# lyclyc52/NeRF_RPN

Hardware: AMD Instinct MI355X
Metric: scenes/sec (160^3x4 grids, VGG19-3D+FPN+RPN fwd+bwd) (higher is better)
Workload: dtype bf16; 1 GPU; configs[1]: one 160x160x160x4 rgb-sigma grid per GPU, VGG19-EF 3D + FPN + anchor RPN (OBB, 16 GT boxes per scene), fwd+bwd+clip+AdamW, random-init weights; scenes_per_gpu=1, parallelism=dp1, world_size_seen=1, backend=single process

## Files before the change

### include/nerfrpn.h

```cpp
#ifndef NERFRPN_H
#define NERFRPN_H

#include <stddef.h>
#include <stdint.h>

#ifdef __cplusplus
extern "C" {
#endif

typedef void *nrpn_stream_t;

enum nrpn_status {
  NRPN_OK = 0,
  NRPN_ERR_ARG = -1,
  NRPN_ERR_LAUNCH = -2,
  NRPN_ERR_DEVICE = -3
};

enum nrpn_dtype { NRPN_F32 = 0, NRPN_BF16 = 1 };

const char *nrpn_last_error(void);
int nrpn_abi_version(void);
int nrpn_check_device(int ordinal);

// ... 233 lines not shown
int nrpn_roipool_obb_bwd(const float *dout, const int32_t *argmax, const float *rois, const int32_t *level_of, int level, int num_rois,
                         float scale, int interpolation, int x, int y, int z, int c, int o0, int o1, int o2, void *dfeat, void *workspace,
                         int dtype, nrpn_stream_t stream);

int nrpn_a2a_reduce_bf16(const void *recv, const float *local, int rank, int world, int64_t chunk, void *out, nrpn_stream_t stream);
int nrpn_grad_sumsq_floats(void);
int nrpn_grad_sumsq(const float *grad, int64_t count, float grad_scale, float *sumsq, nrpn_stream_t stream);
int nrpn_adamw_step(float *param, const float *grad, float *exp_avg, float *exp_avg_sq, int64_t count,
                    const float *sumsq, float grad_scale, float max_norm, float lr, float beta1, float beta2, float eps,
                    float weight_decay, int step, void *shadow_bf16, nrpn_stream_t stream);
int nrpn_adamw_step_zero_grad(float *param, float *grad, float *exp_avg, float *exp_avg_sq, int64_t count,
                              const float *sumsq, float grad_scale, float max_norm, float lr, float beta1, float beta2, float eps,
                              float weight_decay, int step, void *shadow_bf16, nrpn_stream_t stream);
int nrpn_transpose_weights(const float *master, void *dst, const int64_t *table, const int32_t *tile_prefix, int nweights,
                           int total_tiles, int dtype, nrpn_stream_t stream);
int nrpn_reduce_slices(const float *partials, int slices, int64_t count, float *dst, int accumulate, const float *bias_partials,
                       int wrows, int cout, float *gbias, int accumulate_bias, nrpn_stream_t stream);
size_t nrpn_conv3d_wgrad_bias_offset(int n, int gx, int gy, int gz, int ksize);

enum nrpn_heatmap_kernel { NRPN_HEATMAP_GAUSSIAN = 0, NRPN_HEATMAP_BOX = 1 };
int nrpn_heatmap_splat(const int32_t *aabbs, int num_boxes, const double *factors, const int32_t *factor_offsets, int kernel_type,
                       int x, int y, int z, float *out, nrpn_stream_t stream);
int nrpn_gaussian_filter3d(const float *in, int x, int y, int z, float sigma, int radius, const double *weights, float *work, float *out,
                           nrpn_stream_t stream);
int nrpn_heatmap_work_doubles(void);
int nrpn_heatmap_standardize(const float *in, int64_t n, double *work, float *out, float *mean_std, nrpn_stream_t stream);
int nrpn_render_mip(const float *heatmap, int x, int y, int z, int downsample, float value_scale, const double *cams, int num_frames,
                    const double *jet, int width, int height, double *work, uint8_t *rgb, float *mip, nrpn_stream_t stream);

int nrpn_zoom_cubic3d(const float *in, int nx, int ny, int nz, const double *h_zpow, int ox, int oy, int oz, double *coef, float *out,
// ... 68 lines not shown
```

### include/nerfrpn_tools.h

```cpp
#ifndef NERFRPN_TOOLS_H
#define NERFRPN_TOOLS_H
#include "nerfrpn.h"

#ifdef __cplusplus
extern "C" {
#endif

int nrpn_set_conv_kstep_bytes(int kb);
int nrpn_set_conv_lds_dma(int on);
int nrpn_set_conv_tile_m(int bm);
int nrpn_set_conv_halo_auto(int on);
int nrpn_set_conv_halo_pairing(int mode);
int nrpn_set_conv_stagger(int on);
int nrpn_set_conv_big_split(int on);
int nrpn_set_wgrad_big_tile(int on);
int nrpn_set_wgrad_pack2(int on);
int nrpn_set_sumsq_form(int form, int grid);
int nrpn_set_wgrad_transpose_read(int on);
int nrpn_set_rows_big_tile(int on);
int nrpn_set_rows_tail_split(int on);
int nrpn_set_bn_fast(int on);
int nrpn_set_bn_reduce_v8(int on);
int nrpn_set_pool_fast(int on);
int nrpn_set_gn_fast(int on);
int64_t nrpn_fastdiv_host(int64_t n, int64_t d);
int nrpn_set_window_attn_mfma(int on);

#ifdef __cplusplus
}
#endif
#endif
```

### nerf_rpn_amd/csrc/common.h

```cpp
#pragma once
#include <hip/hip_runtime.h>
#include <hip/hip_bf16.h>

#include <cstdarg>
#include <cstdint>
#include <cstdio>

#include "../../include/nerfrpn.h"
#include "../../include/nerfrpn_tools.h"

int nrpn_fail(int code, const char *fmt, ...);

#define NRPN_REQUIRE(cond, ...)                                 \
  do {                                                          \
    if (!(cond)) return nrpn_fail(NRPN_ERR_ARG, __VA_ARGS__);   \
  } while (0)

#define NRPN_HIP(call)                                                                          \
  do {                                                                                          \
    hipError_t e_ = (call);                                                                     \
    if (e_ != hipSuccess) return nrpn_fail(NRPN_ERR_LAUNCH, "%s: %s", #call, hipGetErrorString(e_)); \
  } while (0)

#define NRPN_LAUNCH_CHECK(name)                                                                  \
// ... 11 lines not shown
  unsigned l = 0;
  while ((1ull << l) < d) ++l;
  f.m = (unsigned)((((unsigned long long)1 << (31 + l)) + d - 1) / d);
  f.sh = l - 1;
  return f;
}
__device__ __forceinline__ unsigned fastdiv(unsigned n, const FastDiv &f) { return f.d == 1 ? n : (__umulhi(n, f.m) >> f.sh); }


int nrpn_ensure_dynamic_lds(const void *kernel, int bytes);
#define NRPN_LDS(kernel, bytes)                                                                         \
  do {                                                                                                  \
    if (int rc_ = nrpn_ensure_dynamic_lds(reinterpret_cast<const void *>(kernel), (int)(bytes))) return rc_; \
  } while (0)

static inline hipStream_t as_stream(nrpn_stream_t s) { return reinterpret_cast<hipStream_t>(s); }
static inline int64_t cdiv64(int64_t a, int64_t b) { return (a + b - 1) / b; }

__device__ __forceinline__ float bf16_bits_to_f32(unsigned short h) { return __uint_as_float(((unsigned)h) << 16); }
__device__ __forceinline__ unsigned short f32_to_bf16_bits(float f) { return __builtin_bit_cast(unsigned short, (__bf16)f); }

template <typename T> struct elem;
template <> struct elem<float> {
  static __device__ __forceinline__ float ld(const float *p) { return *p; }
  static __device__ __forceinline__ void st(float *p, float v) { *p = v; }
};
template <> struct elem<unsigned short> {
  static __device__ __forceinline__ float ld(const unsigned short *p) { return bf16_bits_to_f32(*p); }
  static __device__ __forceinline__ void st(unsigned short *p, float v) { *p = f32_to_bf16_bits(v); }
};
// ... 1 lines not shown
```

### nerf_rpn_amd/csrc/conv3d.hip

```cpp
#include "conv_common.cuh"

#ifndef NRPN_HALO_PAIRING_DEFAULT
#define NRPN_HALO_PAIRING_DEFAULT 2
#endif

template <typename T, int BN, int MODE, bool OUTF32, int KB, bool GLDS, int BM = 128, bool ROWS = false>
__global__ void __launch_bounds__(256, BM == 128 ? 2 : 1) conv_igemm_kernel(const ConvArgs p) {
  constexpr int WAVES_N = (BN == 128) ? 2 : 1;
  constexpr int TM = BM / (32 * (4 / WAVES_N));
  constexpr int TN = 2;
  constexpr int KE = KB / (int)sizeof(T);
  constexpr int PPR = KB / 16;
  constexpr int RSTEP = 256 / PPR;
  constexpr int A_RPT = BM / RSTEP;
  constexpr int B_RPT = BN / RSTEP;
  constexpr int SWZ_SH = (KB == 64) ? 2 : 1;
  constexpr int A_BYTES = BM * KB, B_BYTES = BN * KB;
  extern __shared__ __attribute__((aligned(16))) char lds[];

  const int tid = threadIdx.x, lane = tid & 63, wave = tid >> 6;
  const int wm = wave / WAVES_N, wn = wave % WAVES_N;
  const unsigned ntiles = (p.Cout + BN - 1) / BN;
  const unsigned tiles = (unsigned)((p.M + BM - 1) / BM) * ntiles;
  unsigned zsplit, tile;
// ... 1116 lines not shown
template <typename T, bool OUTF32>
__global__ void rows_epilogue_kernel(const float *__restrict__ ws, const float *__restrict__ bias, void *__restrict__ y, long long total,
                                     int cout, int relu, int nslices, const T *__restrict__ mask, const unsigned *__restrict__ rows) {
  for (long long i = (long long)blockIdx.x * blockDim.x + threadIdx.x; i < total; i += (long long)gridDim.x * blockDim.x) {
    float o = ws[i];
    for (int z = 1; z < nslices; ++z) o += ws[z * total + i];
    const long long r = i / cout;
    const int col = (int)(i - r * cout);
    const long long dst = (long long)rows[2 * r] * cout + col;
    o += bias ? bias[col] : 0.f;
    if (relu) o = fmaxf(o, 0.f);
    if (mask && !(elem<T>::ld(mask + dst) > 0.f)) o = 0.f;
    if (OUTF32) reinterpret_cast<float *>(y)[dst] = o;
    else elem<T>::st(reinterpret_cast<T *>(y) + dst, o);
  }
}

struct Knobs {
  int glds;
  int bm;
  int stagger;
  int big_split;
  int kb;
  int dbg;
  int halo_auto;
  int halo_xp;
};
static std::atomic<int> g_conv_glds{1}, g_conv_bm{0}, g_conv_stagger{1}, g_conv_big_split{1}, g_conv_kb{128}, g_conv_halo_auto{1}, g_conv_halo_xp{NRPN_HALO_PAIRING_DEFAULT};
static Knobs resolve_knobs(const nrpn_conv_opts *o, int flags = 0) {
  Knobs k{g_conv_glds.load(std::memory_order_relaxed), g_conv_bm.load(std::memory_order_relaxed), g_conv_stagger.load(std::memory_order_relaxed),
// ... 257 lines not shown
  } else {
    a.ksplit = workspace ? conv_ksplit(a.M, cout, cin, a.taps, es, kn) : 1;
    if (a.ksplit > 1) a.ws = reinterpret_cast<float *>(workspace);
  }
  const int nsl = a.ksplit;
  if (a.ksplit <= 1 && workspace && !segs && !stats && !out_f32 && dtype == NRPN_BF16 && conv_tile_kind(a.M, cout, cin, es, false, false, kn) == 1) {
    const TailSplit t = conv_tail_split(a.M, cout, cin, a.taps, es, kn);
    if (t.ks > 1) { a.tail_tile0 = t.tile0; a.tail_ks = t.ks; a.ws = reinterpret_cast<float *>(workspace); }
  }
  int rc = (dtype == NRPN_F32) ? launch_conv<float, 0>(a, true, st, kn) : launch_conv<bf16s, 0>(a, out_f32, st, kn);
  if (!rc && a.tail_ks > 1) {
    const long long row0 = (long long)a.tail_tile0 * 256, total = (a.M - row0) * cout;
    const int blocks = (int)min((long long)2048, (total + 255) / 256);
    const float *b = (flags & NRPN_CONV_BIAS) ? bias : nullptr;
    const bf16s *mk = a.mask ? reinterpret_cast<const bf16s *>(a.mask) + row0 * cout : nullptr;
    hipLaunchKernelGGL((splitk_epilogue_kernel<bf16s, false>), dim3(blocks), dim3(256), 0, st, a.ws, b, reinterpret_cast<bf16s *>(y) + row0 * cout, total, cout,
                       (flags & NRPN_CONV_RELU) ? 1 : 0, a.tail_ks, mk, a.scale);
    NRPN_LAUNCH_CHECK("splitk_epilogue (tail)");
    return NRPN_OK;
  }
  if (rc || a.ksplit <= 1) return rc;
  const long long total = a.M * cout;
  const int blocks = (int)min((long long)4096, (total + 255) / 256);
  const float *b = (flags & NRPN_CONV_BIAS) ? bias : nullptr;
  const int relu = (flags & NRPN_CONV_RELU) ? 1 : 0;
  if (dtype == NRPN_F32 || out_f32) {
    if (dtype == NRPN_F32) hipLaunchKernelGGL((splitk_epilogue_kernel<float, true>), dim3(blocks), dim3(256), 0, st, a.ws, b, y, total, cout, relu, nsl, (const float *)a.mask, a.scale);
    else hipLaunchKernelGGL((splitk_epilogue_kernel<bf16s, true>), dim3(blocks), dim3(256), 0, st, a.ws, b, y, total, cout, relu, nsl, (const bf16s *)a.mask, a.scale);
  } else {
    hipLaunchKernelGGL((splitk_epilogue_kernel<bf16s, false>), dim3(blocks), dim3(256), 0, st, a.ws, b, y, total, cout, relu, nsl, (const bf16s *)a.mask, a.scale);
  }
  NRPN_LAUNCH_CHECK("splitk_epilogue");
  return NRPN_OK;
}

extern "C" int nrpn_conv3d_fwd(const void *x, const void *wp, const float *bias, void *y, int n, int gx, int gy, int gz, int cin,
                               int cout, int wrows, int ksize, int dtype, int flags, void *workspace, const void *relu_mask,
                               nrpn_stream_t stream) {
  NRPN_REQUIRE(n > 0 && gx > 0 && gy > 0 && gz > 0, "conv3d_fwd: bad sizes");
  NRPN_REQUIRE(!relu_mask || !(flags & NRPN_CONV_OUT_F32) || dtype == NRPN_F32, "conv3d_fwd: relu_mask needs outputs in the input dtype");
  return conv3d_fwd_impl(x, wp, bias, relu_mask, y, (long long)n * gx * gy * gz, gx, gy, gz, nullptr, cin, cout, wrows, ksize, dtype, flags,
                         workspace, stream);
}

static int fwd_stats_rows(long long M, int cin, int cout, int ksize, int dtype, const Knobs &kn, const Grid &g) {
// ... 132 lines not shown
  const size_t lds_ = 2 * (size_t)(128 + 128) * 128;
  int rc;
  if (dtype == NRPN_F32) rc = launch_igemm(conv_igemm_kernel<float, 128, 0, true, 128, true, 128, true>, grid, lds_, st, a);
  else if (out_f32) rc = launch_igemm(conv_igemm_kernel<bf16s, 128, 0, true, 128, true, 128, true>, grid, lds_, st, a);
  else rc = launch_igemm(conv_igemm_kernel<bf16s, 128, 0, false, 128, true, 128, true>, grid, lds_, st, a);
  if (rc) return rc;
  NRPN_LAUNCH_CHECK("conv3d_fwd_rows");
  if (ks > 1 || a.tail_ks > 1) {
    const long long row0 = a.tail_ks > 1 ? (long long)a.tail_tile0 * 128 : 0;
    const int nsl = a.tail_ks > 1 ? a.tail_ks : ks;
    const long long total = (nrows - row0) * cout;
    const int blocks = (int)min((long long)2048, (total + 255) / 256);
    const float *b = (flags & NRPN_CONV_BIAS) ? bias : nullptr;
    const int relu = (flags & NRPN_CONV_RELU) ? 1 : 0;
    const uint32_t *rw = rows + 2 * row0;
    if (dtype == NRPN_F32) hipLaunchKernelGGL((rows_epilogue_kernel<float, true>), dim3(blocks), dim3(256), 0, st, a.ws, b, y, total, cout, relu, nsl, (const float *)relu_mask, rw);
    else if (out_f32) hipLaunchKernelGGL((rows_epilogue_kernel<bf16s, true>), dim3(blocks), dim3(256), 0, st, a.ws, b, y, total, cout, relu, nsl, (const bf16s *)relu_mask, rw);
    else hipLaunchKernelGGL((rows_epilogue_kernel<bf16s, false>), dim3(blocks), dim3(256), 0, st, a.ws, b, y, total, cout, relu, nsl, (const bf16s *)relu_mask, rw);
    NRPN_LAUNCH_CHECK("rows_epilogue");
  }
  return NRPN_OK;
}

static int stem_fwd_impl(const void *x, const void *wp, const float *bias, void *y, int n, int gx, int gy, int gz, int cout,
                         int stride, int dtype, int flags, const nrpn_conv_opts *opts, nrpn_stream_t stream) {
  NRPN_REQUIRE(stride == 1 || stride == 2, "stem: stride must be 1 or 2 (got %d)", stride);
  NRPN_REQUIRE(dtype == NRPN_F32 || dtype == NRPN_BF16, "stem: bad dtype %d", dtype);
  NRPN_REQUIRE(n > 0 && gx > 0 && gy > 0 && gz > 0 && cout > 0, "stem: bad sizes");
  NRPN_REQUIRE(x && wp && y, "stem: null pointer");
  NRPN_REQUIRE(!opts || opts->size == (int32_t)sizeof(nrpn_conv_opts), "stem: opts->size must be sizeof(nrpn_conv_opts)");
  NRPN_REQUIRE(!opts || (!opts->relu_mask && !opts->stats), "stem: relu_mask / stats are not available on the stem");
  ConvArgs a{};
  a.x = x; a.w = wp; a.bias = bias; a.y = y;
// ... 967 lines not shown
}

__global__ void unpack_stem_zrow_kernel(const float *__restrict__ gp, int cout, float *__restrict__ gw, int accumulate, int slices) {
  const long long i = (long long)blockIdx.x * blockDim.x + threadIdx.x;
  if (i >= (long long)cout * 4 * 343) return;
  const int tap = (int)(i % 343), c = (int)((i / 343) % 4), o = (int)(i / (343 * 4));
  const int dz = tap % 7, dxy = tap / 7;
  const float *src = gp + ((long long)dxy * cout + o) * 32 + (dz + 1) * 4 + c;
  const long long st = (long long)49 * cout * 32;
  float v0 = 0.f, v1 = 0.f, v2 = 0.f, v3 = 0.f;
  int s = 0;
  for (; s + 3 < slices; s += 4) { v0 += src[s * st]; v1 += src[(s + 1) * st]; v2 += src[(s + 2) * st]; v3 += src[(s + 3) * st]; }
  for (; s < slices; ++s) v0 += src[s * st];
  const float v = (v0 + v1) + (v2 + v3);
  gw[i] = accumulate ? gw[i] + v : v;
}

static bool stem_zrow_ok(int gz, int cout, int stride) { return stride == 2 && gz % 2 == 0 && cout == 64; }
static int stem_zrow_slices(long long M, int elem_bytes) {
  const long long chunks = (M + (elem_bytes == 2 ? 64 : 32) - 1) / (elem_bytes == 2 ? 64 : 32);
  long long s = 73;
  if (s > chunks / 8) s = chunks / 8;
  if (s < 1) s = 1;
  const long long per = (chunks + s - 1) / s;
  return (int)((chunks + per - 1) / per);
}

__global__ void bias_finalize_kernel(const float *__restrict__ part, int slices, int wrows, int cout, float *__restrict__ gbias, int accumulate) {
  const int c = blockIdx.x * blockDim.x + threadIdx.x;
  if (c >= cout) return;
// ... 358 lines not shown

__global__ void unpack_stem_wgrad_kernel(const float *__restrict__ gp, int cout, int kpad, float *__restrict__ gw, int accumulate, int slices) {
  const long long i = (long long)blockIdx.x * blockDim.x + threadIdx.x;
  if (i >= (long long)cout * 4 * 343) return;
  const int tap = (int)(i % 343), c = (int)((i / 343) % 4), o = (int)(i / (343 * 4));
  const float *src = gp + (long long)o * kpad + tap * 4 + c;
  float v = 0.f;
  for (int s = 0; s < slices; ++s) v += src[(long long)s * cout * kpad];
  gw[i] = accumulate ? gw[i] + v : v;
}

extern "C" int nrpn_unpack_stem_wgrad(const float *gw_packed, int cout, int dtype, float *gw_ref, int accumulate, int slices,
                                      int64_t slice_floats, nrpn_stream_t stream) {
  NRPN_REQUIRE(gw_packed && gw_ref && cout > 0 && slices > 0, "unpack_stem_wgrad: bad args");
  if (slice_floats == (int64_t)49 * cout * 32) {
    hipLaunchKernelGGL(unpack_stem_zrow_kernel, dim3((unsigned)cdiv64((long long)cout * 4 * 343, 256)), dim3(256), 0, as_stream(stream), gw_packed,
                       cout, gw_ref, accumulate, slices);
    NRPN_LAUNCH_CHECK("unpack_stem_zrow");
    return NRPN_OK;
  }
  const int kpad = nrpn_stem_kpad(dtype);
  hipLaunchKernelGGL(unpack_stem_wgrad_kernel, dim3((unsigned)cdiv64((long long)cout * 4 * 343, 256)), dim3(256), 0, as_stream(stream),
                     gw_packed, cout, kpad, gw_ref, accumulate, slices);
  NRPN_LAUNCH_CHECK("unpack_stem_wgrad");
  return NRPN_OK;
}
```

### nerf_rpn_amd/csrc/elementwise.hip

```cpp
#include "common.h"
#include <atomic>

typedef unsigned short bf16s;
typedef __attribute__((ext_vector_type(4))) float f4;
typedef __attribute__((ext_vector_type(4))) unsigned short us4;

template <typename T> struct vec4;
template <> struct vec4<float> {
  static __device__ __forceinline__ f4 ld(const float *p) { return *reinterpret_cast<const f4 *>(p); }
  static __device__ __forceinline__ void st(float *p, f4 v) { *reinterpret_cast<f4 *>(p) = v; }
};
template <> struct vec4<bf16s> {
  static __device__ __forceinline__ f4 ld(const bf16s *p) {
    const us4 u = *reinterpret_cast<const us4 *>(p);
    f4 v = {bf16_bits_to_f32(u[0]), bf16_bits_to_f32(u[1]), bf16_bits_to_f32(u[2]), bf16_bits_to_f32(u[3])};
    return v;
  }
  static __device__ __forceinline__ void st(bf16s *p, f4 v) {
    typedef __attribute__((ext_vector_type(4))) __bf16 b4;
    *reinterpret_cast<us4 *>(p) = __builtin_bit_cast(us4, __builtin_convertvector(v, b4));
  }
};

template <typename T, int V> struct vecv;
// ... 1358 lines not shown

extern "C" int nrpn_adamw_step(float *param, const float *grad, float *exp_avg, float *exp_avg_sq, int64_t count, const float *sumsq,
                               float grad_scale, float max_norm, float lr, float beta1, float beta2, float eps, float weight_decay, int step,
                               void *shadow_bf16, nrpn_stream_t stream) {
  return adamw_launch(param, const_cast<float *>(grad), exp_avg, exp_avg_sq, count, sumsq, grad_scale, max_norm, lr, beta1, beta2, eps, weight_decay, step,
                      shadow_bf16, false, stream);
}

extern "C" int nrpn_adamw_step_zero_grad(float *param, float *grad, float *exp_avg, float *exp_avg_sq, int64_t count, const float *sumsq,
                                         float grad_scale, float max_norm, float lr, float beta1, float beta2, float eps, float weight_decay,
                                         int step, void *shadow_bf16, nrpn_stream_t stream) {
  return adamw_launch(param, grad, exp_avg, exp_avg_sq, count, sumsq, grad_scale, max_norm, lr, beta1, beta2, eps, weight_decay, step, shadow_bf16, true,
                      stream);
}

template <typename T>
__global__ void __launch_bounds__(256) transpose_weights_kernel(const float *__restrict__ master, T *__restrict__ dst, const long long *__restrict__ table,
                                                                const int *__restrict__ tile_prefix, int nweights) {
  __shared__ float tile[64][65];
  const int job = blockIdx.x;
  int lo = 0, hi = nweights - 1;
  while (lo < hi) {
    const int mid = (lo + hi + 1) >> 1;
    if (tile_prefix[mid] <= job) lo = mid; else hi = mid - 1;
  }
  const long long off = table[lo * 4];
  const int taps = (int)table[lo * 4 + 1], cout = (int)table[lo * 4 + 2], cin = (int)table[lo * 4 + 3];
  int j = job - tile_prefix[lo];
  const int tn = (cin + 63) / 64, tm = (cout + 63) / 64;
  const int c0 = (j % tn) * 64; j /= tn;
  const int o0 = (j % tm) * 64; j /= tm;
  const int tap = j;
  const float *src = master + off + (long long)tap * cout * cin;
  T *out = dst + off + (long long)(taps - 1 - tap) * cin * cout;
  const int tx = threadIdx.x & 63, ty = threadIdx.x >> 6;
  for (int r = ty; r < 64; r += 4)
    tile[r][tx] = (o0 + r < cout && c0 + tx < cin) ? src[(long long)(o0 + r) * cin + c0 + tx] : 0.f;
  __syncthreads();
  for (int r = ty; r < 64; r += 4)
    if (c0 + r < cin && o0 + tx < cout) elem<T>::st(out + (long long)(c0 + r) * cout + o0 + tx, tile[tx][r]);
}

extern "C" int nrpn_transpose_weights(const float *master, void *dst, const int64_t *table, const int32_t *tile_prefix, int nweights,
                                      int total_tiles, int dtype, nrpn_stream_t stream) {
  NRPN_REQUIRE(master && dst && table && tile_prefix && nweights > 0 && total_tiles > 0, "transpose_weights: bad args");
  NRPN_REQUIRE(dtype == NRPN_F32 || dtype == NRPN_BF16, "transpose_weights: bad dtype %d", dtype);
  hipStream_t st = as_stream(stream);
  if (dtype == NRPN_F32)
    hipLaunchKernelGGL(transpose_weights_kernel<float>, dim3(total_tiles), dim3(256), 0, st, master, (float *)dst, (const long long *)table, tile_prefix, nweights);
  else
    hipLaunchKernelGGL(transpose_weights_kernel<bf16s>, dim3(total_tiles), dim3(256), 0, st, master, (bf16s *)dst, (const long long *)table, tile_prefix, nweights);
  NRPN_LAUNCH_CHECK("transpose_weights");
  return NRPN_OK;
}

__global__ void __launch_bounds__(256) reduce_slices_kernel(const float *__restrict__ part, int slices, long long count4, long long stride4,
                                                            float *__restrict__ dst, int accumulate, const float *__restrict__ bias_part,
                                                            int wrows, int cout, float *__restrict__ gbias, int accumulate_bias) {
  if (bias_part && blockIdx.x == gridDim.x - 1) {
    for (int c = threadIdx.x; c < cout; c += 256) {
      float s = 0.f;
      for (int k = 0; k < slices; ++k) s += bias_part[(long long)k * wrows + c];
      gbias[c] = accumulate_bias ? gbias[c] + s : s;
    }
    return;
  }
  const f4 *p4 = reinterpret_cast<const f4 *>(part);
  f4 *d4 = reinterpret_cast<f4 *>(dst);
  const long long nb = gridDim.x - (bias_part ? 1 : 0);
  for (long long i = (long long)blockIdx.x * blockDim.x + threadIdx.x; i < count4; i += nb * blockDim.x) {
    f4 a = p4[i];
    for (int s = 1; s < slices; ++s) { const f4 b = p4[(long long)s * stride4 + i]; a[0] += b[0]; a[1] += b[1]; a[2] += b[2]; a[3] += b[3]; }
    if (accumulate) { const f4 o = d4[i]; a[0] += o[0]; a[1] += o[1]; a[2] += o[2]; a[3] += o[3]; }
    d4[i] = a;
  }
}

extern "C" int nrpn_reduce_slices(const float *partials, int slices, int64_t count, float *dst, int accumulate, const float *bias_partials,
                                  int wrows, int cout, float *gbias, int accumulate_bias, nrpn_stream_t stream) {
  NRPN_REQUIRE(partials && dst && slices > 0 && count > 0 && count % 4 == 0, "reduce_slices: count must be a positive multiple of 4");
  NRPN_REQUIRE(((reinterpret_cast<uintptr_t>(partials) | reinterpret_cast<uintptr_t>(dst)) & 15) == 0, "reduce_slices: 16-byte alignment required");
  NRPN_REQUIRE(!bias_partials || (gbias && cout > 0 && wrows >= cout), "reduce_slices: bad bias arguments");
  hipLaunchKernelGGL(reduce_slices_kernel, dim3(ew_blocks(count / 4) + (bias_partials ? 1 : 0)), dim3(256), 0, as_stream(stream), partials, slices,
                     (long long)(count / 4), (long long)(count / 4), dst, accumulate, bias_partials, wrows, cout, gbias, accumulate_bias);
  NRPN_LAUNCH_CHECK("reduce_slices");
  return NRPN_OK;
}

template <typename S, typename T>
__global__ void ingest_kernel(const S *__restrict__ src, T *__restrict__ dst, long long voxels, int mode) {
  for (long long v = (long long)blockIdx.x * blockDim.x + threadIdx.x; v < voxels; v += (long long)gridDim.x * blockDim.x) {
    float c[4];
#pragma unroll
    for (int k = 0; k < 4; ++k) c[k] = sizeof(S) == 1 ? (float)src[v * 4 + k] * (1.0f / 255.0f) : (float)src[v * 4 + k];
    if (mode == 1) c[3] = fminf(fmaxf(1.0f - expf(-expf(c[3]) / 100.0f), 0.f), 1.f);
    else if (mode == 2) c[3] = fminf(fmaxf(1.0f - expf(-fmaxf(c[3], 0.f) / 100.0f), 0.f), 1.f);
    f4 o = {c[0], c[1], c[2], c[3]};
    vec4<T>::st(dst + v * 4, o);
  }
// ... 106 lines not shown
```

### nerf_rpn_amd/ops.py

```python
import itertools
import math
from types import SimpleNamespace

import torch

from . import lib
from .lib import BF16, CONV_BIAS, CONV_OUT_F32, CONV_RELU, F32, call

_QCACHE = {"epoch": -1, "map": {}}


def query(name, *args):
    if _QCACHE["epoch"] != lib.KNOB_EPOCH[0]:
        _QCACHE["epoch"], _QCACHE["map"] = lib.KNOB_EPOCH[0], {}
    m = _QCACHE["map"]
    key = (name, args)
    v = m.get(key)
    if v is None:
        v = m[key] = lib.query(name, *args)
    return v


def _query_opts(name, opts, *args):
    if _QCACHE["epoch"] != lib.KNOB_EPOCH[0]:
# ... 486 lines not shown
            self.trans[dtype] = ent
        if ent[1] != self.epoch:
            self._transpose(dtype)
        return ent[0][off:off + taps * cout * cin].view(taps, cin, cout)

    def _transpose(self, dtype):
        ent = self.trans[dtype]
        if self.table is None:
            rows, prefix = [], [0]
            for (o, t, co, ci, _) in self.entries:
                rows.append([o, t, co, ci])
                prefix.append(prefix[-1] + t * ((co + 63) // 64) * ((ci + 63) // 64))
            dev = self.master.device
            self.table = (torch.tensor(rows, dtype=torch.int64, device=dev), torch.tensor(prefix, dtype=torch.int32, device=dev), prefix[-1])
        tab, prefix, total = self.table
        call("transpose_weights", _p(self.master), _p(ent[0]), _p(tab), _p(prefix), len(self.entries), total, F32 if dtype == torch.float32 else BF16, _s())
        self.launches["transpose"] += 1
        ent[1] = self.epoch

    def prefetch_dgrad(self):
        side = _wgrad_side_stream(self.master.device)
        if side is None or not self.trans or self.table is None:
            return
        side.wait_stream(torch.cuda.current_stream(self.master.device))
        with torch.cuda.stream(side):
            for dtype in list(self.trans):
                if self.trans[dtype][1] != self.epoch:
                    self._transpose(dtype)
            ev = torch.cuda.Event()
            ev.record(side)
        _DGRAD_READY["event"] = ev
# ... 2030 lines not shown
```

Baseline: 115.2 scenes/sec.

## Add batched-load fast paths for split-K epilogues, slice reduction, and weight transpose

Adds new kernels that sum split-K slices by issuing up to eight independent vector loads per batch before accumulating. They cover the conv split-K and rows epilogues, the wgrad reduce_slices (two outputs per thread, used only when slices exceed a threshold), and the stem z-row unpack, now indexed per packed element. The weight transpose gains a vectorized fast kernel and can read from the bf16 shadow copy instead of the fp32 master when it is current, halving the bytes read. All paths sit behind a runtime mask that is on by default. The aim is to raise memory-level parallelism on bandwidth-bound reductions, at the cost of more registers, more code paths and possible changes in summation order.

```diff
diff --git a/include/nerfrpn.h b/include/nerfrpn.h
--- a/include/nerfrpn.h
+++ b/include/nerfrpn.h
@@ -271,6 +271,9 @@
                               float weight_decay, int step, void *shadow_bf16, nrpn_stream_t stream);
 int nrpn_transpose_weights(const float *master, void *dst, const int64_t *table, const int32_t *tile_prefix, int nweights,
                            int total_tiles, int dtype, nrpn_stream_t stream);
+int nrpn_transpose_weights_bf16(const void *shadow, void *dst, const int64_t *table, const int32_t *tile_prefix, int nweights,
+                                int total_tiles, nrpn_stream_t stream);
+int64_t nrpn_slice_sum_fast_launches(int part);
 int nrpn_reduce_slices(const float *partials, int slices, int64_t count, float *dst, int accumulate, const float *bias_partials,
                        int wrows, int cout, float *gbias, int accumulate_bias, nrpn_stream_t stream);
 size_t nrpn_conv3d_wgrad_bias_offset(int n, int gx, int gy, int gz, int ksize);
diff --git a/include/nerfrpn_tools.h b/include/nerfrpn_tools.h
--- a/include/nerfrpn_tools.h
+++ b/include/nerfrpn_tools.h
@@ -23,6 +23,8 @@
 int nrpn_set_bn_reduce_v8(int on);
 int nrpn_set_pool_fast(int on);
 int nrpn_set_gn_fast(int on);
+int nrpn_set_slice_sum_fast(int mask);
+int nrpn_set_reduce_slices_fast_min(int slices);
 int64_t nrpn_fastdiv_host(int64_t n, int64_t d);
 int nrpn_set_window_attn_mfma(int on);
 
diff --git a/nerf_rpn_amd/csrc/common.h b/nerf_rpn_amd/csrc/common.h
--- a/nerf_rpn_amd/csrc/common.h
+++ b/nerf_rpn_amd/csrc/common.h
@@ -2,6 +2,7 @@
 #include <hip/hip_runtime.h>
 #include <hip/hip_bf16.h>
 
+#include <atomic>
 #include <cstdarg>
 #include <cstdint>
 #include <cstdio>
@@ -49,6 +50,11 @@
     if (int rc_ = nrpn_ensure_dynamic_lds(reinterpret_cast<const void *>(kernel), (int)(bytes))) return rc_; \
   } while (0)
 
+extern std::atomic<int> g_slice_sum_fast;
+extern std::atomic<long long> g_slice_sum_launches[4];
+static inline bool slice_sum_fast_on(int part) { return (g_slice_sum_fast.load(std::memory_order_relaxed) >> part) & 1; }
+static inline void slice_sum_fast_count(int part) { g_slice_sum_launches[part].fetch_add(1, std::memory_order_relaxed); }
+
 static inline hipStream_t as_stream(nrpn_stream_t s) { return reinterpret_cast<hipStream_t>(s); }
 static inline int64_t cdiv64(int64_t a, int64_t b) { return (a + b - 1) / b; }
 
diff --git a/nerf_rpn_amd/csrc/conv3d.hip b/nerf_rpn_amd/csrc/conv3d.hip
--- a/nerf_rpn_amd/csrc/conv3d.hip
+++ b/nerf_rpn_amd/csrc/conv3d.hip
@@ -1154,6 +1154,129 @@
     if (OUTF32) reinterpret_cast<float *>(y)[dst] = o;
     else elem<T>::st(reinterpret_cast<T *>(y) + dst, o);
   }
+}
+
+std::atomic<int> g_slice_sum_fast{15};
+std::atomic<long long> g_slice_sum_launches[4];
+extern "C" int nrpn_set_slice_sum_fast(int mask) { g_slice_sum_fast = mask & 15; return NRPN_OK; }
+extern "C" int64_t nrpn_slice_sum_fast_launches(int part) {
+  return part >= 0 && part < 4 ? (int64_t)g_slice_sum_launches[part].load(std::memory_order_relaxed) : -1;
+}
+
+template <int Q, int N>
+__device__ __forceinline__ void slice_batch(const float *__restrict__ ws, unsigned idx, unsigned total, int z, f4 (&acc)[Q]) {
+  f4 buf[N][Q];
+#pragma unroll
+  for (int u = 0; u < N; ++u)
+#pragma unroll
+    for (int q = 0; q < Q; ++q) buf[u][q] = *reinterpret_cast<const f4 *>(ws + ((unsigned)(z + u) * total + idx + q * 4));
+#pragma unroll
+  for (int u = 0; u < N; ++u)
+#pragma unroll
+    for (int q = 0; q < Q; ++q) acc[q] = (u == 0 && z == 0) ? buf[u][q] : acc[q] + buf[u][q];
+}
+template <int Q>
+__device__ __forceinline__ void slice_sum(const float *__restrict__ ws, unsigned idx, unsigned total, int nslices, f4 (&acc)[Q]) {
+  for (int z = 0; z < nslices; z += 8) {
+    switch (min(nslices - z, 8)) {
+      case 1: slice_batch<Q, 1>(ws, idx, total, z, acc); break;
+      case 2: slice_batch<Q, 2>(ws, idx, total, z, acc); break;
+      case 3: slice_batch<Q, 3>(ws, idx, total, z, acc); break;
+      case 4: slice_batch<Q, 4>(ws, idx, total, z, acc); break;
+      case 5: slice_batch<Q, 5>(ws, idx, total, z, acc); break;
+      case 6: slice_batch<Q, 6>(ws, idx, total, z, acc); break;
+      case 7: slice_batch<Q, 7>(ws, idx, total, z, acc); break;
+      default: slice_batch<Q, 8>(ws, idx, total, z, acc); break;
+    }
+  }
+}
+
+template <typename T, bool OUTF32, bool ROWS>
+__global__ void __launch_bounds__(256) slice_epilogue_fast_kernel(const float *__restrict__ ws, const float *__restrict__ bias, void *__restrict__ y,
+                                                                  unsigned pieces, int cout, int relu, int nslices, const T *__restrict__ mask,
+                                                                  const float *__restrict__ scale, const unsigned *__restrict__ rows, FastDiv dv,
+                                                                  int hoist) {
+  constexpr int V = OUTF32 ? 4 : 8, Q = V / 4;
+  typedef __attribute__((ext_vector_type(V))) unsigned short usv;
+  const unsigned total = pieces * V, stride = gridDim.x * 256u, cpr = dv.d;
+  const bool pow2 = (cpr & (cpr - 1)) == 0;
+  f4 bi[Q], sc[Q];
+#pragma unroll
+  for (int q = 0; q < Q; ++q) { bi[q] = f4{0.f, 0.f, 0.f, 0.f}; sc[q] = f4{1.f, 1.f, 1.f, 1.f}; }
+  unsigned p = blockIdx.x * 256u + threadIdx.x;
+  if (hoist) {
+    const unsigned col = (pow2 ? (p & (cpr - 1)) : (p - fastdiv(p, dv) * cpr)) * V;
+#pragma unroll
+    for (int q = 0; q < Q; ++q) {
+      if (bias) bi[q] = *reinterpret_cast<const f4 *>(bias + col + q * 4);
+      if (scale) sc[q] = *reinterpret_cast<const f4 *>(scale + col + q * 4);
+    }
+  }
+  for (; p < pieces; p += stride) {
+    unsigned r = 0, colp;
+    if (ROWS || !pow2) r = fastdiv(p, dv);
+    colp = pow2 ? (p & (cpr - 1)) : (p - r * cpr);
+    const unsigned dst = ROWS ? rows[2 * r] * (unsigned)cout + colp * V : p * V;
+    usv mb;
+    f4 mf;
+    if (mask) {
+      if (sizeof(T) == 2) mb = *reinterpret_cast<const usv *>(mask + dst);
+      else mf = *reinterpret_cast<const f4 *>(mask + dst);
+    }
+    if (!hoist) {
+#pragma unroll
+      for (int q = 0; q < Q; ++q) {
+        if (bias) bi[q] = *reinterpret_cast<const f4 *>(bias + colp * V + q * 4);
+        if (scale) sc[q] = *reinterpret_cast<const f4 *>(scale + colp * V + q * 4);
+      }
+    }
+    f4 acc[Q];
+#pragma unroll
+    for (int q = 0; q < Q; ++q) acc[q] = f4{0.f, 0.f, 0.f, 0.f};
+    slice_sum<Q>(ws, p * V, total, nslices, acc);
+    float o[V];
+    {
+#pragma clang fp contract(off)
+#pragma unroll
+      for (int k = 0; k < V; ++k) {
+        float v = acc[k / 4][k % 4];
+        if (scale) v *= sc[k / 4][k % 4];
+        v += bi[k / 4][k % 4];
+        if (relu) v = fmaxf(v, 0.f);
+        if (mask) {
+          const float m = sizeof(T) == 2 ? bf16_bits_to_f32(mb[k]) : mf[k % 4];
+          if (!(m > 0.f)) v = 0.f;
+        }
+        o[k] = v;
+      }
+    }
+    if (OUTF32) {
+      *reinterpret_cast<f4 *>(reinterpret_cast<float *>(y) + dst) = f4{o[0], o[1], o[2], o[3]};
+    } else {
+      typedef __attribute__((ext_vector_type(V))) float fv;
+      typedef __attribute__((ext_vector_type(V))) __bf16 bv;
+      fv w;
+#pragma unroll
+      for (int k = 0; k < V; ++k) w[k] = o[k];
+      *reinterpret_cast<usv *>(reinterpret_cast<bf16s *>(y) + dst) = __builtin_bit_cast(usv, __builtin_convertvector(w, bv));
+    }
+  }
+}
+
+template <typename T, bool OUTF32, bool ROWS>
+static bool slice_epilogue_fast(const float *ws, const float *bias, void *y, long long total, int cout, int relu, int nsl, const T *mask,
+                                const float *scale, const unsigned *rows, hipStream_t st) {
+  constexpr int V = OUTF32 ? 4 : 8;
+  if (!slice_sum_fast_on(0) || cout % V || total <= 0 || (long long)nsl * total >= (1ll << 31)) return false;
+  if ((reinterpret_cast<uintptr_t>(ws) | reinterpret_cast<uintptr_t>(bias) | reinterpret_cast<uintptr_t>(y) | reinterpret_cast<uintptr_t>(mask) |
+       reinterpret_cast<uintptr_t>(scale)) & 15) return false;
+  const long long pieces = total / V;
+  const int blocks = (int)min((long long)2048, (pieces + 255) / 256);
+  const int hoist = ((long long)blocks * 256) % (cout / V) == 0;
+  hipLaunchKernelGGL((slice_epilogue_fast_kernel<T, OUTF32, ROWS>), dim3(blocks), dim3(256), 0, st, ws, bias, y, (unsigned)pieces, cout, relu, nsl, mask, scale,
+                     rows, make_fastdiv((unsigned)(cout / V)), hoist);
+  slice_sum_fast_count(0);
+  return true;
 }
 
 struct Knobs {
@@ -1441,8 +1564,10 @@
     const int blocks = (int)min((long long)2048, (total + 255) / 256);
     const float *b = (flags & NRPN_CONV_BIAS) ? bias : nullptr;
     const bf16s *mk = a.mask ? reinterpret_cast<const bf16s *>(a.mask) + row0 * cout : nullptr;
-    hipLaunchKernelGGL((splitk_epilogue_kernel<bf16s, false>), dim3(blocks), dim3(256), 0, st, a.ws, b, reinterpret_cast<bf16s *>(y) + row0 * cout, total, cout,
-                       (flags & NRPN_CONV_RELU) ? 1 : 0, a.tail_ks, mk, a.scale);
+    if (!slice_epilogue_fast<bf16s, false, false>(a.ws, b, reinterpret_cast<bf16s *>(y) + row0 * cout, total, cout, (flags & NRPN_CONV_RELU) ? 1 : 0, a.tail_ks,
+                                                  mk, a.scale, nullptr, st))
+      hipLaunchKernelGGL((splitk_epilogue_kernel<bf16s, false>), dim3(blocks), dim3(256), 0, st, a.ws, b, reinterpret_cast<bf16s *>(y) + row0 * cout, total, cout,
+                         (flags & NRPN_CONV_RELU) ? 1 : 0, a.tail_ks, mk, a.scale);
     NRPN_LAUNCH_CHECK("splitk_epilogue (tail)");
     return NRPN_OK;
   }
@@ -1451,11 +1576,15 @@
   const int blocks = (int)min((long long)4096, (total + 255) / 256);
   const float *b = (flags & NRPN_CONV_BIAS) ? bias : nullptr;
   const int relu = (flags & NRPN_CONV_RELU) ? 1 : 0;
-  if (dtype == NRPN_F32 || out_f32) {
-    if (dtype == NRPN_F32) hipLaunchKernelGGL((splitk_epilogue_kernel<float, true>), dim3(blocks), dim3(256), 0, st, a.ws, b, y, total, cout, relu, nsl, (const float *)a.mask, a.scale);
-    else hipLaunchKernelGGL((splitk_epilogue_kernel<bf16s, true>), dim3(blocks), dim3(256), 0, st, a.ws, b, y, total, cout, relu, nsl, (const bf16s *)a.mask, a.scale);
+  if (dtype == NRPN_F32) {
+    if (!slice_epilogue_fast<float, true, false>(a.ws, b, y, total, cout, relu, nsl, (const float *)a.mask, a.scale, nullptr, st))
+      hipLaunchKernelGGL((splitk_epilogue_kernel<float, true>), dim3(blocks), dim3(256), 0, st, a.ws, b, y, total, cout, relu, nsl, (const float *)a.mask, a.scale);
+  } else if (out_f32) {
+    if (!slice_epilogue_fast<bf16s, true, false>(a.ws, b, y, total, cout, relu, nsl, (const bf16s *)a.mask, a.scale, nullptr, st))
+      hipLaunchKernelGGL((splitk_epilogue_kernel<bf16s, true>), dim3(blocks), dim3(256), 0, st, a.ws, b, y, total, cout, relu, nsl, (const bf16s *)a.mask, a.scale);
   } else {
-    hipLaunchKernelGGL((splitk_epilogue_kernel<bf16s, false>), dim3(blocks), dim3(256), 0, st, a.ws, b, y, total, cout, relu, nsl, (const bf16s *)a.mask, a.scale);
+    if (!slice_epilogue_fast<bf16s, false, false>(a.ws, b, y, total, cout, relu, nsl, (const bf16s *)a.mask, a.scale, nullptr, st))
+      hipLaunchKernelGGL((splitk_epilogue_kernel<bf16s, false>), dim3(blocks), dim3(256), 0, st, a.ws, b, y, total, cout, relu, nsl, (const bf16s *)a.mask, a.scale);
   }
   NRPN_LAUNCH_CHECK("splitk_epilogue");
   return NRPN_OK;
@@ -1618,9 +1747,16 @@
     const float *b = (flags & NRPN_CONV_BIAS) ? bias : nullptr;
     const int relu = (flags & NRPN_CONV_RELU) ? 1 : 0;
     const uint32_t *rw = rows + 2 * row0;
-    if (dtype == NRPN_F32) hipLaunchKernelGGL((rows_epilogue_kernel<float, true>), dim3(blocks), dim3(256), 0, st, a.ws, b, y, total, cout, relu, nsl, (const float *)relu_mask, rw);
-    else if (out_f32) hipLaunchKernelGGL((rows_epilogue_kernel<bf16s, true>), dim3(blocks), dim3(256), 0, st, a.ws, b, y, total, cout, relu, nsl, (const bf16s *)relu_mask, rw);
-    else hipLaunchKernelGGL((rows_epilogue_kernel<bf16s, false>), dim3(blocks), dim3(256), 0, st, a.ws, b, y, total, cout, relu, nsl, (const bf16s *)relu_mask, rw);
+    if (dtype == NRPN_F32) {
+      if (!slice_epilogue_fast<float, true, true>(a.ws, b, y, total, cout, relu, nsl, (const float *)relu_mask, nullptr, rw, st))
+        hipLaunchKernelGGL((rows_epilogue_kernel<float, true>), dim3(blocks), dim3(256), 0, st, a.ws, b, y, total, cout, relu, nsl, (const float *)relu_mask, rw);
+    } else if (out_f32) {
+      if (!slice_epilogue_fast<bf16s, true, true>(a.ws, b, y, total, cout, relu, nsl, (const bf16s *)relu_mask, nullptr, rw, st))
+        hipLaunchKernelGGL((rows_epilogue_kernel<bf16s, true>), dim3(blocks), dim3(256), 0, st, a.ws, b, y, total, cout, relu, nsl, (const bf16s *)relu_mask, rw);
+    } else {
+      if (!slice_epilogue_fast<bf16s, false, true>(a.ws, b, y, total, cout, relu, nsl, (const bf16s *)relu_mask, nullptr, rw, st))
+        hipLaunchKernelGGL((rows_epilogue_kernel<bf16s, false>), dim3(blocks), dim3(256), 0, st, a.ws, b, y, total, cout, relu, nsl, (const bf16s *)relu_mask, rw);
+    }
     NRPN_LAUNCH_CHECK("rows_epilogue");
   }
   return NRPN_OK;
@@ -2618,6 +2754,23 @@
   for (; s < slices; ++s) v0 += src[s * st];
   const float v = (v0 + v1) + (v2 + v3);
   gw[i] = accumulate ? gw[i] + v : v;
+}
+
+__global__ void __launch_bounds__(256) unpack_stem_zrow_fast_kernel(const float *__restrict__ gp, int cout, float *__restrict__ gw, int accumulate, int slices) {
+  const unsigned i = blockIdx.x * 256u + threadIdx.x;
+  if (i >= 49u * cout * 32u) return;
+  const unsigned j = i & 31, row = i >> 5;
+  if (j < 4) return;
+  const unsigned o = row % (unsigned)cout, dxy = row / (unsigned)cout, dz = (j >> 2) - 1, c = j & 3;
+  const float *src = gp + i;
+  const long long st = (long long)49 * cout * 32;
+  float v0 = 0.f, v1 = 0.f, v2 = 0.f, v3 = 0.f;
+  int s = 0;
+  for (; s + 3 < slices; s += 4) { v0 += src[s * st]; v1 += src[(s + 1) * st]; v2 += src[(s + 2) * st]; v3 += src[(s + 3) * st]; }
+  for (; s < slices; ++s) v0 += src[s * st];
+  const float v = (v0 + v1) + (v2 + v3);
+  float *out = gw + ((long long)o * 4 + c) * 343 + dxy * 7 + dz;
+  *out = accumulate ? *out + v : v;
 }
 
 static bool stem_zrow_ok(int gz, int cout, int stride) { return stride == 2 && gz % 2 == 0 && cout == 64; }
@@ -3006,8 +3159,14 @@
                                       int64_t slice_floats, nrpn_stream_t stream) {
   NRPN_REQUIRE(gw_packed && gw_ref && cout > 0 && slices > 0, "unpack_stem_wgrad: bad args");
   if (slice_floats == (int64_t)49 * cout * 32) {
-    hipLaunchKernelGGL(unpack_stem_zrow_kernel, dim3((unsigned)cdiv64((long long)cout * 4 * 343, 256)), dim3(256), 0, as_stream(stream), gw_packed,
-                       cout, gw_ref, accumulate, slices);
+    if (slice_sum_fast_on(3) && cout < (1 << 20)) {
+      hipLaunchKernelGGL(unpack_stem_zrow_fast_kernel, dim3((unsigned)cdiv64((long long)49 * cout * 32, 256)), dim3(256), 0, as_stream(stream), gw_packed,
+                         cout, gw_ref, accumulate, slices);
+      slice_sum_fast_count(3);
+    } else {
+      hipLaunchKernelGGL(unpack_stem_zrow_kernel, dim3((unsigned)cdiv64((long long)cout * 4 * 343, 256)), dim3(256), 0, as_stream(stream), gw_packed,
+                         cout, gw_ref, accumulate, slices);
+    }
     NRPN_LAUNCH_CHECK("unpack_stem_zrow");
     return NRPN_OK;
   }
diff --git a/nerf_rpn_amd/csrc/elementwise.hip b/nerf_rpn_amd/csrc/elementwise.hip
--- a/nerf_rpn_amd/csrc/elementwise.hip
+++ b/nerf_rpn_amd/csrc/elementwise.hip
@@ -1396,31 +1396,119 @@
                       stream);
 }
 
-template <typename T>
-__global__ void __launch_bounds__(256) transpose_weights_kernel(const float *__restrict__ master, T *__restrict__ dst, const long long *__restrict__ table,
-                                                                const int *__restrict__ tile_prefix, int nweights) {
-  __shared__ float tile[64][65];
+struct TransJob { long long off; int taps, cout, cin, tap, o0, c0; };
+__device__ __forceinline__ TransJob trans_job(const long long *__restrict__ table, const int *__restrict__ tile_prefix, int nweights) {
   const int job = blockIdx.x;
   int lo = 0, hi = nweights - 1;
   while (lo < hi) {
     const int mid = (lo + hi + 1) >> 1;
     if (tile_prefix[mid] <= job) lo = mid; else hi = mid - 1;
   }
-  const long long off = table[lo * 4];
-  const int taps = (int)table[lo * 4 + 1], cout = (int)table[lo * 4 + 2], cin = (int)table[lo * 4 + 3];
+  TransJob t;
+  t.off = table[lo * 4];
+  t.taps = (int)table[lo * 4 + 1]; t.cout = (int)table[lo * 4 + 2]; t.cin = (int)table[lo * 4 + 3];
   int j = job - tile_prefix[lo];
-  const int tn = (cin + 63) / 64, tm = (cout + 63) / 64;
-  const int c0 = (j % tn) * 64; j /= tn;
-  const int o0 = (j % tm) * 64; j /= tm;
-  const int tap = j;
-  const float *src = master + off + (long long)tap * cout * cin;
-  T *out = dst + off + (long long)(taps - 1 - tap) * cin * cout;
+  const int tn = (t.cin + 63) / 64, tm = (t.cout + 63) / 64;
+  t.c0 = (j % tn) * 64; j /= tn;
+  t.o0 = (j % tm) * 64; j /= tm;
+  t.tap = j;
+  return t;
+}
+
+template <typename S, typename T>
+__global__ void __launch_bounds__(256) transpose_weights_kernel(const S *__restrict__ master, T *__restrict__ dst, const long long *__restrict__ table,
+                                                                const int *__restrict__ tile_prefix, int nweights) {
+  __shared__ float tile[64][65];
+  const TransJob t = trans_job(table, tile_prefix, nweights);
+  const int cout = t.cout, cin = t.cin, o0 = t.o0, c0 = t.c0;
+  const S *src = master + t.off + (long long)t.tap * cout * cin;
+  T *out = dst + t.off + (long long)(t.taps - 1 - t.tap) * cin * cout;
   const int tx = threadIdx.x & 63, ty = threadIdx.x >> 6;
   for (int r = ty; r < 64; r += 4)
-    tile[r][tx] = (o0 + r < cout && c0 + tx < cin) ? src[(long long)(o0 + r) * cin + c0 + tx] : 0.f;
+    tile[r][tx] = (o0 + r < cout && c0 + tx < cin) ? elem<S>::ld(src + (long long)(o0 + r) * cin + c0 + tx) : 0.f;
   __syncthreads();
   for (int r = ty; r < 64; r += 4)
     if (c0 + r < cin && o0 + tx < cout) elem<T>::st(out + (long long)(c0 + r) * cout + o0 + tx, tile[tx][r]);
+}
+
+template <typename S>
+__global__ void __launch_bounds__(256) transpose_weights_fast_kernel(const S *__restrict__ master, bf16s *__restrict__ dst, const long long *__restrict__ table,
+                                                                     const int *__restrict__ tile_prefix, int nweights, int aligned) {
+  typedef __attribute__((ext_vector_type(8))) unsigned short us8;
+  typedef __attribute__((ext_vector_type(4))) unsigned u4;
+  constexpr int PD = 33, P = 2 * PD;
+  __shared__ unsigned tile32[64 * PD];
+  bf16s *tile = reinterpret_cast<bf16s *>(tile32);
+  const TransJob t = trans_job(table, tile_prefix, nweights);
+  const int cout = t.cout, cin = t.cin, o0 = t.o0, c0 = t.c0;
+  const S *src = master + t.off + (long long)t.tap * cout * cin;
+  bf16s *out = dst + t.off + (long long)(t.taps - 1 - t.tap) * cin * cout;
+  if (aligned && !((cin | cout | (int)t.off) & 7)) {
+    const int lr = threadIdx.x >> 3, l8 = (threadIdx.x & 7) * 8;
+#pragma unroll
+    for (int h = 0; h < 2; ++h) {
+      const int r = lr + h * 32;
+      u4 w = {0u, 0u, 0u, 0u};
+      if (o0 + r < cout && c0 + l8 < cin) {
+        const S *p = src + (long long)(o0 + r) * cin + c0 + l8;
+        if (sizeof(S) == 2) {
+          w = *reinterpret_cast<const u4 *>(p);
+        } else {
+          typedef __attribute__((ext_vector_type(8))) float f8;
+          typedef __attribute__((ext_vector_type(8))) __bf16 b8;
+          const f4 x0 = *reinterpret_cast<const f4 *>(p), x1 = *reinterpret_cast<const f4 *>(p + 4);
+          const f8 x = {x0[0], x0[1], x0[2], x0[3], x1[0], x1[1], x1[2], x1[3]};
+          w = __builtin_bit_cast(u4, __builtin_convertvector(x, b8));
+        }
+      }
+      unsigned *row = tile32 + r * PD + (l8 >> 1);
+      row[0] = w[0]; row[1] = w[1]; row[2] = w[2]; row[3] = w[3];
+    }
+    __syncthreads();
+#pragma unroll
+    for (int h = 0; h < 2; ++h) {
+      const int c = lr + h * 32;
+      if (c0 + c < cin && o0 + l8 < cout) {
+        us8 v;
+#pragma unroll
+        for (int k = 0; k < 8; ++k) v[k] = tile[(l8 + k) * P + c];
+        *reinterpret_cast<us8 *>(out + (long long)(c0 + c) * cout + o0 + l8) = v;
+      }
+    }
+    return;
+  }
+  const int tx = threadIdx.x & 63, ty = threadIdx.x >> 6;
+  for (int r = ty; r < 64; r += 4)
+    tile[r * P + tx] = (o0 + r < cout && c0 + tx < cin) ? f32_to_bf16_bits(elem<S>::ld(src + (long long)(o0 + r) * cin + c0 + tx)) : (bf16s)0;
+  __syncthreads();
+  for (int r = ty; r < 64; r += 4)
+    if (c0 + r < cin && o0 + tx < cout) out[(long long)(c0 + r) * cout + o0 + tx] = tile[tx * P + r];
+}
+
+__global__ void __launch_bounds__(256) transpose_weights_f32_fast_kernel(const float *__restrict__ master, float *__restrict__ dst, const long long *__restrict__ table,
+                                                                         const int *__restrict__ tile_prefix, int nweights, int aligned) {
+  __shared__ float tile[64][65];
+  const TransJob t = trans_job(table, tile_prefix, nweights);
+  const int cout = t.cout, cin = t.cin, o0 = t.o0, c0 = t.c0;
+  const float *src = master + t.off + (long long)t.tap * cout * cin;
+  float *out = dst + t.off + (long long)(t.taps - 1 - t.tap) * cin * cout;
+  const int tx = threadIdx.x & 63, ty = threadIdx.x >> 6;
+  if (aligned && !((cin | (int)t.off) & 3)) {
+    const int lr = threadIdx.x >> 4, l4 = (threadIdx.x & 15) * 4;
+#pragma unroll
+    for (int h = 0; h < 4; ++h) {
+      const int r = lr + h * 16;
+      f4 v = {0.f, 0.f, 0.f, 0.f};
+      if (o0 + r < cout && c0 + l4 < cin) v = *reinterpret_cast<const f4 *>(src + (long long)(o0 + r) * cin + c0 + l4);
+      tile[r][l4] = v[0]; tile[r][l4 + 1] = v[1]; tile[r][l4 + 2] = v[2]; tile[r][l4 + 3] = v[3];
+    }
+  } else {
+    for (int r = ty; r < 64; r += 4)
+      tile[r][tx] = (o0 + r < cout && c0 + tx < cin) ? src[(long long)(o0 + r) * cin + c0 + tx] : 0.f;
+  }
+  __syncthreads();
+  for (int r = ty; r < 64; r += 4)
+    if (c0 + r < cin && o0 + tx < cout) out[(long long)(c0 + r) * cout + o0 + tx] = tile[tx][r];
 }
 
 extern "C" int nrpn_transpose_weights(const float *master, void *dst, const int64_t *table, const int32_t *tile_prefix, int nweights,
@@ -1428,25 +1516,52 @@
   NRPN_REQUIRE(master && dst && table && tile_prefix && nweights > 0 && total_tiles > 0, "transpose_weights: bad args");
   NRPN_REQUIRE(dtype == NRPN_F32 || dtype == NRPN_BF16, "transpose_weights: bad dtype %d", dtype);
   hipStream_t st = as_stream(stream);
-  if (dtype == NRPN_F32)
-    hipLaunchKernelGGL(transpose_weights_kernel<float>, dim3(total_tiles), dim3(256), 0, st, master, (float *)dst, (const long long *)table, tile_prefix, nweights);
-  else
-    hipLaunchKernelGGL(transpose_weights_kernel<bf16s>, dim3(total_tiles), dim3(256), 0, st, master, (bf16s *)dst, (const long long *)table, tile_prefix, nweights);
+  const int aligned = ((reinterpret_cast<uintptr_t>(master) | reinterpret_cast<uintptr_t>(dst)) & 15) == 0;
+  const long long *tab = reinterpret_cast<const long long *>(table);
+  if (slice_sum_fast_on(2)) {
+    if (dtype == NRPN_F32)
+      hipLaunchKernelGGL(transpose_weights_f32_fast_kernel, dim3(total_tiles), dim3(256), 0, st, master, (float *)dst, tab, tile_prefix, nweights, aligned);
+    else
+      hipLaunchKernelGGL(transpose_weights_fast_kernel<float>, dim3(total_tiles), dim3(256), 0, st, master, (bf16s *)dst, tab, tile_prefix, nweights, aligned);
+    slice_sum_fast_count(2);
+  } else if (dtype == NRPN_F32) {
+    hipLaunchKernelGGL((transpose_weights_kernel<float, float>), dim3(total_tiles), dim3(256), 0, st, master, (float *)dst, tab, tile_prefix, nweights);
+  } else {
+    hipLaunchKernelGGL((transpose_weights_kernel<float, bf16s>), dim3(total_tiles), dim3(256), 0, st, master, (bf16s *)dst, tab, tile_prefix, nweights);
+  }
   NRPN_LAUNCH_CHECK("transpose_weights");
   return NRPN_OK;
+}
+
+extern "C" int nrpn_transpose_weights_bf16(const void *shadow, void *dst, const int64_t *table, const int32_t *tile_prefix, int nweights,
+                                           int total_tiles, nrpn_stream_t stream) {
+  NRPN_REQUIRE(shadow && dst && table && tile_prefix && nweights > 0 && total_tiles > 0, "transpose_weights_bf16: bad args");
+  hipStream_t st = as_stream(stream);
+  const int aligned = ((reinterpret_cast<uintptr_t>(shadow) | reinterpret_cast<uintptr_t>(dst)) & 15) == 0;
+  const long long *tab = reinterpret_cast<const long long *>(table);
+  if (slice_sum_fast_on(2)) {
+    hipLaunchKernelGGL(transpose_weights_fast_kernel<bf16s>, dim3(total_tiles), dim3(256), 0, st, (const bf16s *)shadow, (bf16s *)dst, tab, tile_prefix, nweights, aligned);
+    slice_sum_fast_count(2);
+  } else {
+    hipLaunchKernelGGL((transpose_weights_kernel<bf16s, bf16s>), dim3(total_tiles), dim3(256), 0, st, (const bf16s *)shadow, (bf16s *)dst, tab, tile_prefix, nweights);
+  }
+  NRPN_LAUNCH_CHECK("transpose_weights_bf16");
+  return NRPN_OK;
+}
+
+__device__ __forceinline__ void reduce_slices_bias(const float *__restrict__ bias_part, int slices, int wrows, int cout, float *__restrict__ gbias,
+                                                   int accumulate_bias) {
+  for (int c = threadIdx.x; c < cout; c += 256) {
+    float s = 0.f;
+    for (int k = 0; k < slices; ++k) s += bias_part[(long long)k * wrows + c];
+    gbias[c] = accumulate_bias ? gbias[c] + s : s;
+  }
 }
 
 __global__ void __launch_bounds__(256) reduce_slices_kernel(const float *__restrict__ part, int slices, long long count4, long long stride4,
                                                             float *__restrict__ dst, int accumulate, const float *__restrict__ bias_part,
                                                             int wrows, int cout, float *__restrict__ gbias, int accumulate_bias) {
-  if (bias_part && blockIdx.x == gridDim.x - 1) {
-    for (int c = threadIdx.x; c < cout; c += 256) {
-      float s = 0.f;
-      for (int k = 0; k < slices; ++k) s += bias_part[(long long)k * wrows + c];
-      gbias[c] = accumulate_bias ? gbias[c] + s : s;
-    }
-    return;
-  }
+  if (bias_part && blockIdx.x == gridDim.x - 1) { reduce_slices_bias(bias_part, slices, wrows, cout, gbias, accumulate_bias); return; }
   const f4 *p4 = reinterpret_cast<const f4 *>(part);
   f4 *d4 = reinterpret_cast<f4 *>(dst);
   const long long nb = gridDim.x - (bias_part ? 1 : 0);
@@ -1458,13 +1573,63 @@
   }
 }
 
+static std::atomic<int> g_reduce_fast_min{32};
+extern "C" int nrpn_set_reduce_slices_fast_min(int slices) { g_reduce_fast_min = slices < 1 ? 1 : slices; return NRPN_OK; }
+template <int N>
+__device__ __forceinline__ void reduce_batch(const f4 *__restrict__ p4, long long stride4, long long ia, long long ib, int z, f4 &a, f4 &b) {
+  f4 ba[N], bb[N];
+#pragma unroll
+  for (int u = 0; u < N; ++u) { ba[u] = p4[(long long)(z + u) * stride4 + ia]; bb[u] = p4[(long long)(z + u) * stride4 + ib]; }
+#pragma unroll
+  for (int u = 0; u < N; ++u) {
+    a = (u == 0 && z == 0) ? ba[u] : a + ba[u];
+    b = (u == 0 && z == 0) ? bb[u] : b + bb[u];
+  }
+}
+
+__global__ void __launch_bounds__(256) reduce_slices_fast_kernel(const float *__restrict__ part, int slices, long long count4, long long stride4,
+                                                                 float *__restrict__ dst, int accumulate, const float *__restrict__ bias_part,
+                                                                 int wrows, int cout, float *__restrict__ gbias, int accumulate_bias) {
+  if (bias_part && blockIdx.x == gridDim.x - 1) { reduce_slices_bias(bias_part, slices, wrows, cout, gbias, accumulate_bias); return; }
+  const f4 *p4 = reinterpret_cast<const f4 *>(part);
+  f4 *d4 = reinterpret_cast<f4 *>(dst);
+  const long long stride = (long long)(gridDim.x - (bias_part ? 1 : 0)) * 256;
+  for (long long i = (long long)blockIdx.x * 256 + threadIdx.x; i < count4; i += 2 * stride) {
+    const bool two = i + stride < count4;
+    const long long j = two ? i + stride : i;
+    f4 oa = {0.f, 0.f, 0.f, 0.f}, ob = oa, a = oa, b = oa;
+    if (accumulate) { oa = d4[i]; ob = d4[j]; }
+    for (int z = 0; z < slices; z += 8) {
+      switch (min(slices - z, 8)) {
+        case 1: reduce_batch<1>(p4, stride4, i, j, z, a, b); break;
+        case 2: reduce_batch<2>(p4, stride4, i, j, z, a, b); break;
+        case 3: reduce_batch<3>(p4, stride4, i, j, z, a, b); break;
+        case 4: reduce_batch<4>(p4, stride4, i, j, z, a, b); break;
+        case 5: reduce_batch<5>(p4, stride4, i, j, z, a, b); break;
+        case 6: reduce_batch<6>(p4, stride4, i, j, z, a, b); break;
+        case 7: reduce_batch<7>(p4, stride4, i, j, z, a, b); break;
+        default: reduce_batch<8>(p4, stride4, i, j, z, a, b); break;
+      }
+    }
+    if (accumulate) { a = a + oa; b = b + ob; }
+    d4[i] = a;
+    if (two) d4[j] = b;
+  }
+}
+
 extern "C" int nrpn_reduce_slices(const float *partials, int slices, int64_t count, float *dst, int accumulate, const float *bias_partials,
                                   int wrows, int cout, float *gbias, int accumulate_bias, nrpn_stream_t stream) {
   NRPN_REQUIRE(partials && dst && slices > 0 && count > 0 && count % 4 == 0, "reduce_slices: count must be a positive multiple of 4");
   NRPN_REQUIRE(((reinterpret_cast<uintptr_t>(partials) | reinterpret_cast<uintptr_t>(dst)) & 15) == 0, "reduce_slices: 16-byte alignment required");
   NRPN_REQUIRE(!bias_partials || (gbias && cout > 0 && wrows >= cout), "reduce_slices: bad bias arguments");
-  hipLaunchKernelGGL(reduce_slices_kernel, dim3(ew_blocks(count / 4) + (bias_partials ? 1 : 0)), dim3(256), 0, as_stream(stream), partials, slices,
-                     (long long)(count / 4), (long long)(count / 4), dst, accumulate, bias_partials, wrows, cout, gbias, accumulate_bias);
+  if (slice_sum_fast_on(1) && slices >= g_reduce_fast_min.load(std::memory_order_relaxed)) {
+    hipLaunchKernelGGL(reduce_slices_fast_kernel, dim3(ew_blocks((count / 4 + 1) / 2) + (bias_partials ? 1 : 0)), dim3(256), 0, as_stream(stream), partials, slices,
+                       (long long)(count / 4), (long long)(count / 4), dst, accumulate, bias_partials, wrows, cout, gbias, accumulate_bias);
+    slice_sum_fast_count(1);
+  } else {
+    hipLaunchKernelGGL(reduce_slices_kernel, dim3(ew_blocks(count / 4) + (bias_partials ? 1 : 0)), dim3(256), 0, as_stream(stream), partials, slices,
+                       (long long)(count / 4), (long long)(count / 4), dst, accumulate, bias_partials, wrows, cout, gbias, accumulate_bias);
+  }
   NRPN_LAUNCH_CHECK("reduce_slices");
   return NRPN_OK;
 }
diff --git a/nerf_rpn_amd/ops.py b/nerf_rpn_amd/ops.py
--- a/nerf_rpn_amd/ops.py
+++ b/nerf_rpn_amd/ops.py
@@ -524,7 +524,10 @@
             dev = self.master.device
             self.table = (torch.tensor(rows, dtype=torch.int64, device=dev), torch.tensor(prefix, dtype=torch.int32, device=dev), prefix[-1])
         tab, prefix, total = self.table
-        call("transpose_weights", _p(self.master), _p(ent[0]), _p(tab), _p(prefix), len(self.entries), total, F32 if dtype == torch.float32 else BF16, _s())
+        if dtype == torch.bfloat16 and self.shadow is not None and self.shadow_epoch == self.epoch:
+            call("transpose_weights_bf16", _p(self.shadow), _p(ent[0]), _p(tab), _p(prefix), len(self.entries), total, _s())
+        else:
+            call("transpose_weights", _p(self.master), _p(ent[0]), _p(tab), _p(prefix), len(self.entries), total, F32 if dtype == torch.float32 else BF16, _s())
         self.launches["transpose"] += 1
         ent[1] = self.epoch
 
```

New measurement: 115.8 scenes/sec, median of 6. About the same (+0.5%).
